# Woody5962/Ranked-List-Truncation

Measured on AMD Instinct MI355X. Metric: ranked-lists/sec (fwd+bwd) at len=300; F1@k vs CPU ref, higher is better.
Workload: dtype f32 (operands, accumulation, storage); products by exact 3xbf16 split, 6 MFMA products, per-product error < 2^-23; 1 GPU; AttnCut + DivLoss(js,f1,augmented) [BASELINE configs[1]], batch 4096 lists/GPU x len 300, full train step incl. Adam and cut metrics; global_batch=4096, seq_len=300, parallelism=dp1

## Files before the change

include/rlt_hip.h:

```cpp
#ifndef RLT_HIP_H
#define RLT_HIP_H

#include <stddef.h>
#include <stdint.h>

#ifdef __cplusplus
extern "C" {
#endif

#define RLT_E_ARG      (-1)
#define RLT_E_SHAPE    (-2)
#define RLT_E_WORKSPACE (-3)
#define RLT_E_ALIGN    (-4)

#define RLT_ABI_VERSION 5
int rlt_abi_version(void);
#define RLT_PRECISION_DEFAULT (-1)
#define RLT_PRECISION_FP32   0
#define RLT_PRECISION_BF16X3 1
#define RLT_PRECISION_BF16X6 2
int rlt_set_precision(int mode);
int rlt_get_precision(void);
const char* rlt_error_string(int code);

// ... 41 lines not shown
                        int32_t* k_out, float* r_k, float* r_best, int32_t* best_k, double* sums,
                        const void* dcg_table, void* ws, size_t ws_bytes, void* stream);

size_t rlt_reward_eval_workspace(int B, int S, int T);
int rlt_reward_eval(const float* labels, const rlt_reward_spec* spec, const float* r_in, int B, int S,
                    const int32_t* k_in, int T, int allow_empty, const void* dcg_table, int accumulate,
                    float* r_at, int32_t* better, float* best, int32_t* best_k,
                    double* curve, double* best_hist, double* sums,
                    void* ws, size_t ws_bytes, void* stream);

size_t rlt_mt_terms_workspace(int B, int S);
int rlt_mt_terms(const float* rerank, const float* cls, const float* labels, int B, int S, float margin,
                 float* terms, void* ws, size_t ws_bytes, void* stream);
int rlt_mt_terms_bwd(const float* cls, const float* labels, const float* terms, int B, int S,
                     float w_rerank, float w_class, const float* gscale,
                     float* d_rerank, float* d_class, void* stream);
int rlt_weighted_sum(const float* const* x, const float* w, int n, float* out, void* stream);

int rlt_cut_metrics(const float* p, const float* labels, const int32_t* k_in, int B, int S,
                    int32_t* k_out, double* f1_out, double* dcg_out, double* sums, void* stream);
int rlt_cut_metrics_ex(const float* p, const float* labels, const int32_t* k_in, int B, int S, double penalty,
                       int32_t* k_out, double* f1_out, double* dcg_out, double* sums, void* stream);

int rlt_task_metrics(const float* labels, const float* pred, int B, int S,
                     double* dcg_out, double* auc_out, double* sums, void* stream);

size_t rlt_truncation_curves_workspace(int B, int S);
int rlt_truncation_curves(const float* labels, int B, int S, double penalty, const void* dcg_table, int accumulate,
                          double* curves, double* best_f1, int32_t* best_f1_k, double* best_dcg, int32_t* best_dcg_k,
                          double* sums, void* ws, size_t ws_bytes, void* stream);

#define RLT_CUT_ARGMAX 0
#define RLT_CUT_PAIR   1
size_t rlt_cut_report_workspace(int B, int S);
int rlt_cut_report(const float* p, int rule, const float* labels, const float* dcg_coef, int B, int S, int metric, float penalty,
                   double metric_penalty, double tau, double sharpen, const void* dcg_table, int accumulate,
                   int32_t* k, float* p_k, float* margin, double* f1, double* dcg, double* best_f1, int32_t* best_f1_k,
                   double* best_dcg, int32_t* best_dcg_k, int32_t* better, double* hist, double* pred_curve, double* reward_curve,
                   double* sums, void* ws, size_t ws_bytes, void* stream);

#define RLT_SWEEP_QUANTILE    0
#define RLT_SWEEP_FIRST_BELOW 1
#define RLT_SWEEP_FIRST_ABOVE 2
#define RLT_SWEEP_COLS        8
size_t rlt_cut_sweep_workspace(int B, int S, int T);
int rlt_cut_sweep(const float* v, int v_stride, int rule, const double* thresholds, int T,
                  const float* labels, int B, int S, double metric_penalty, double beta,
                  const void* dcg_table, int accumulate,
                  int32_t* k , double* curve ,
                  void* ws, size_t ws_bytes, void* stream);

#define RLT_GEMM_RELU       1
#define RLT_GEMM_ACCUMULATE 2
size_t rlt_gemm_workspace(int ta, int tb, int M, int N, int K);
int rlt_gemm(int ta, int tb, int M, int N, int K,
             const float* A, int lda, const float* B, int ldb, float* C, int ldc,
             const float* bias, const float* bias2, int flags,
             void* ws, size_t ws_bytes, int precision, void* stream);
int rlt_gemm_ex(int ta, int tb, int M, int N, int K,
                const float* A, int lda, const float* B, int ldb, float* C, int ldc,
                const float* bias, const float* bias2, int flags,
                const float* relu_mask, int ldmask, float mask_scale, float* colsum_a,
                float drop_p, uint32_t seed,
                void* ws, size_t ws_bytes, int precision, void* stream);

#define RLT_GEMM_NONE   0
#define RLT_GEMM_F32    1
#define RLT_GEMM_3      2
#define RLT_GEMM_3B     3
#define RLT_GEMM_6      4
#define RLT_GEMM_6B     5
#define RLT_GEMM_6C     6
#define RLT_GEMM_6E     7
#define RLT_GEMM_6S     8
typedef struct rlt_gemm_dispatch {
    int family, ta, tb, fast, persistent, ns, kchunk, slab_xcd, epilogue, narrow;
} rlt_gemm_dispatch;
int rlt_gemm_last_dispatch(rlt_gemm_dispatch* out);
#define RLT_GEMM_PTR_A         1
#define RLT_GEMM_PTR_B         2
#define RLT_GEMM_PTR_C         4
#define RLT_GEMM_PTR_BIAS      8
#define RLT_GEMM_PTR_BIAS2     16
#define RLT_GEMM_PTR_BITS_OUT  32
#define RLT_GEMM_PTR_BITS_IN   64
#define RLT_GEMM_PTR_RELU_MASK 128
#define RLT_GEMM_PTR_COLSUM    256
typedef struct rlt_gemm_call {
    int ta, tb, M, N, K, lda, ldb, ldc, flags;
    int aligned16, present, drop, ws_null;
    size_t ws_bytes;
} rlt_gemm_call;
int rlt_gemm_plan(const rlt_gemm_call* call, int precision, rlt_gemm_dispatch* out);

size_t rlt_gemm_bits_words(int M, int N);
int rlt_gemm_bits(int ta, int tb, int M, int N, int K,
                  const float* A, int lda, const float* B, int ldb, float* C, int ldc,
                  const float* bias, int flags, float drop_p, uint32_t seed,
                  uint32_t* relu_bits_out, const uint32_t* mask_bits_in, float mask_scale,
                  int precision, void* stream);
size_t rlt_colsum_workspace(int T, int N);
int rlt_colsum(const float* X, int ldx, int T, int N, float* out, int accumulate,
               void* ws, size_t ws_bytes, void* stream);
int rlt_segment_colsum(const float* X, int ldx, int G, int R, int N, float* out, int ldo,
                       int accumulate, void* stream);

// ... 283 lines not shown
```

ranked-list-truncation_amd/csrc/gemm.hip:

```cpp
#include "common.h"
#include "gemm6s.h"
#include "gemm_plan.h"
#include "split6.h"
#include <type_traits>

namespace {

constexpr int BM = 128, BN = 128, LDT = 132;

struct GemmArgs {
    const float* A; const float* B; float* C;
    const float* bias; const float* bias2;
    int M, N, K, lda, ldb, ldc;
    int vecA, vecB;
    int flags;
    int kchunk;
    float* slab;
    int tiles_m, tiles_n;
    const float* mask; int ldmask;
    float* colsum;
    float* cs_slab;
    float drop_p; uint32_t drop_thr, seed;
    float mask_scale;
    int slab_xcd;
// ... 1238 lines not shown
    __syncthreads();

    int u = 0;
    int nslot = 0; (void)nslot;
    while (true) {
        for (int ti = 0; ti < nt; ++ti) {
            const int b0 = u, b1 = u == 2 ? 0 : u + 1, b2 = b1 == 2 ? 0 : b1 + 1;
            RLT_G6C_STAMP(nslot, 0);
            slot(BoolTag<false>{}, b0, 0, 0, false, 0);
            RLT_G6C_STAMP(nslot, 1);
            __syncthreads();
            RLT_G6C_STAMP(nslot, 2);
            ++nslot;
            RLT_G6C_STAMP(nslot, 0);
            slot(BoolTag<true>{}, b1, b2, b0, ti + 1 < nt || has_next, ti + 2);
            RLT_G6C_STAMP(nslot, 1);
            __syncthreads();
            RLT_G6C_STAMP(nslot, 2);
            ++nslot;
            u = b2;
        }
#ifdef RLT_G6C_NOSTORE
        if (acc[0][0][0] == 123.456f)
#endif
        write_output_t<4>(g, acc, m0 + wm * 64, n0 + wn * 128, true, l31, hh, zslab);
        if (!PERSIST || !has_next) break;
        m0 = nm0; n0 = nn0;
        decode_next();
#pragma unroll
        for (int i = 0; i < 2; ++i)
#pragma unroll
            for (int j = 0; j < 4; ++j)
#pragma unroll
                for (int r = 0; r < 16; ++r) acc[i][j][r] = 0.f;
    }
    if (want_cs) {
        float4* red = reinterpret_cast<float4*>(gsm);
        __syncthreads();
        red[tid] = csum;
        __syncthreads();
        if (tid < 64) {
            float4 t = red[4 * tid];
#pragma unroll
            for (int j = 1; j < 8; ++j) {
                const float4 o = red[(j >> 2) * 256 + 4 * tid + (j & 3)];
                t.x += o.x; t.y += o.y; t.z += o.z; t.w += o.w;
            }
            float* dst = (g.cs_slab ? g.cs_slab + (size_t)zslab * g.M : g.colsum) + m0 + 4 * tid;
            dst[0] = t.x; dst[1] = t.y; dst[2] = t.z; dst[3] = t.w;
        }
    }
}

template <bool KC>
__device__ __forceinline__ size_t off6e(int tid, int ld) {
    if (KC) return (size_t)phys6(tid >> 2) * ld + 4 * (tid & 3);
    return (size_t)(4 * (tid & 3)) * ld + 4 * (tid >> 2);
}
template <bool KC>
__device__ __forceinline__ void load6e(const float* __restrict__ P, int ld, int i, float4& v) {
    v = *reinterpret_cast<const float4*>(P + (size_t)(KC ? 64 * i : i) * ld);
}
template <bool KC>
__device__ __forceinline__ int dst6e(int tid, int p) {
    const int x = tid & 3;
    const int pr = KC ? (tid >> 2) + 64 * p : ((((tid >> 2) * 4) & ~15) | (p << 2) | ((tid >> 2) & 3));
    return pr * 16 + 8 * ((x >> 1) ^ ((pr >> 3) & 1)) + 4 * (x & 1);
}
template <bool KC>
__device__ __forceinline__ void vals6e(const float4 (&v)[4], int p, float& a, float& b, float& c, float& d) {
    if (KC) { a = v[p].x; b = v[p].y; c = v[p].z; d = v[p].w; }
    else {
        const float* f0 = reinterpret_cast<const float*>(&v[0]);
        const float* f1 = reinterpret_cast<const float*>(&v[1]);
        const float* f2 = reinterpret_cast<const float*>(&v[2]);
        const float* f3 = reinterpret_cast<const float*>(&v[3]);
        a = f0[p]; b = f1[p]; c = f2[p]; d = f3[p];
    }
}

template <int NJ>
__device__ __forceinline__ void write_output_simple(const GemmArgs& g, const f32x16 (&acc)[2][NJ], int rbase, int cbase, int l31, int hh, int z) {
    const bool to_slab = g.slab != nullptr;
    float* out = to_slab ? g.slab + (size_t)z * g.M * g.N : g.C;
    const int ldo = to_slab ? g.N : g.ldc;
    const int rb = __builtin_amdgcn_readfirstlane(rbase), cb = __builtin_amdgcn_readfirstlane(cbase);
    const int loff = 4 * hh * ldo + l31;
    const bool relu = !to_slab && (g.flags & RLT_GEMM_RELU), accum = !to_slab && (g.flags & RLT_GEMM_ACCUMULATE);
#pragma unroll
    for (int j = 0; j < NJ; ++j) {
        const int col = cb + j * 32 + l31;
        float bv = 0.f;
        if (!to_slab) {
            if (g.bias) bv += g.bias[col];
            if (g.bias2) bv += g.bias2[col];
        }
#pragma unroll
        for (int i = 0; i < 2; ++i) {
#pragma unroll
            for (int r = 0; r < 16; ++r) {
                const int dr = (r & 3) + 8 * (r >> 2);
                float* base = out + (size_t)(rb + i * 32 + dr) * ldo + (cb + j * 32);
                float v = acc[i][j][r] + bv;
                if (accum) v += base[loff];
                if (relu) v = fmaxf(v, 0.f);
                base[loff] = v;
            }
        }
    }
}

template <bool TA, bool TB, bool PERSIST>
__global__ __launch_bounds__(256, 1) void gemm6e_kernel(GemmArgs g) {
    extern __shared__ __attribute__((aligned(16))) float gsm[];
    uint16_t* lds = reinterpret_cast<uint16_t*>(gsm);
    const int tid = threadIdx.x, lane = tid & 63, wv = __builtin_amdgcn_readfirstlane(tid >> 6);
    const int l31 = lane & 31, hh = lane >> 5;
    const int wm = wv >> 1, wn = wv & 1;
    int bid, zslab;
    decode_block(g, bid, zslab);
    const int tm = bid / g.tiles_n, tn = bid - tm * g.tiles_n;
    int m0 = tm * BM2, n0 = tn * BN2;
    const int kbeg = zslab * g.kchunk;
    const int kend = min(g.K, kbeg + g.kchunk);
    const int nks = (kend - kbeg) / 16;

    f32x16 acc[2][2][4];
#pragma unroll
    for (int i = 0; i < 4; ++i)
#pragma unroll
        for (int j = 0; j < 4; ++j)
#pragma unroll
            for (int r = 0; r < 16; ++r) acc[i >> 1][i & 1][j][r] = 0.f;

    constexpr bool AKC = !TA, BKC = TB;
    const bool want_cs = TA && g.colsum != nullptr && tn == 0;
    float4 csum = make_float4(0.f, 0.f, 0.f, 0.f);
    const int pl = phys6(l31);
    const int csw = 8 * (hh ^ ((pl >> 3) & 1));
    const int arow = (wm * 128 + pl) * 16 + csw, brow = 3 * HB6 + (wn * 128 + pl) * 16 + csw;
    const size_t offA = off6e<AKC>(tid, g.lda), offB = off6e<BKC>(tid, g.ldb);
    int dA[4], dB[4];
#pragma unroll
    for (int p = 0; p < 4; ++p) { dA[p] = dst6e<AKC>(tid, p); dB[p] = 3 * HB6 + dst6e<BKC>(tid, p); }

    int vid = blockIdx.x, nm0 = m0, nn0 = n0;
    bool has_next = false;
    auto decode_next = [&]() {
        const int nwg = g.tiles_m * g.tiles_n;
        vid += gridDim.x;
        has_next = PERSIST && vid < nwg;
        if (has_next) {
            const int q = nwg >> 3, r = nwg & 7, xcd = vid & 7, jj = vid >> 3;
            const int nb = (xcd < r ? xcd * (q + 1) : r * (q + 1) + (xcd - r) * q) + jj;
            const int ntm = nb / g.tiles_n;
            nm0 = ntm * BM2; nn0 = (nb - ntm * g.tiles_n) * BN2;
        }
    };
    auto srcA = [&](int ks) {
        const bool wrap = PERSIST && has_next && ks >= nks;
        const int k0 = kbeg + 16 * (wrap ? ks - nks : min(ks, nks - 1)), mm = wrap ? nm0 : m0;
        return g.A + (AKC ? (size_t)mm * g.lda + k0 : (size_t)k0 * g.lda + mm) + offA;
    };
    auto srcB = [&](int ks) {
        const bool wrap = PERSIST && has_next && ks >= nks;
        const int k0 = kbeg + 16 * (wrap ? ks - nks : min(ks, nks - 1)), nn = wrap ? nn0 : n0;
        return g.B + (BKC ? (size_t)nn * g.ldb + k0 : (size_t)k0 * g.ldb + nn) + offB;
    };
    float4 ra[2][4], rb[2][4];
    auto add_cs = [&](const float4 (&v)[4]) {
#pragma unroll
        for (int i = 0; i < 4; ++i) { csum.x += v[i].x; csum.y += v[i].y; csum.z += v[i].z; csum.w += v[i].w; }
    };
    auto stash_all = [&](uint16_t* wb, const float4 (&va)[4], const float4 (&vb)[4]) {
#pragma unroll
        for (int p = 0; p < 4; ++p) {
            float a, b, c, d;
            uint2 hi, mid, lo;
            vals6e<AKC>(va, p, a, b, c, d);
            split4x3(a, b, c, d, hi, mid, lo);
            *reinterpret_cast<uint2*>(wb + dA[p]) = hi;
            *reinterpret_cast<uint2*>(wb + dA[p] + HB6) = mid;
            *reinterpret_cast<uint2*>(wb + dA[p] + 2 * HB6) = lo;
            vals6e<BKC>(vb, p, a, b, c, d);
            split4x3(a, b, c, d, hi, mid, lo);
            *reinterpret_cast<uint2*>(wb + dB[p]) = hi;
            *reinterpret_cast<uint2*>(wb + dB[p] + HB6) = mid;
            *reinterpret_cast<uint2*>(wb + dB[p] + 2 * HB6) = lo;
        }
    };
    bf16x8 a[4][3], b[2][3];
    auto frag_a = [&](const uint16_t* base, int i, int q) { a[i][q] = *reinterpret_cast<const bf16x8*>(base + arow + q * HB6 + i * 32 * 16); };
    auto frag_b = [&](const uint16_t* base, int j, int q) { b[j & 1][q] = *reinterpret_cast<const bf16x8*>(base + brow + q * HB6 + j * 32 * 16); };

    {
        const float* pa = srcA(0); const float* pb = srcB(0);
#pragma unroll
        for (int i = 0; i < 4; ++i) { load6e<AKC>(pa, g.lda, i, ra[0][i]); load6e<BKC>(pb, g.ldb, i, rb[0][i]); }
        pa = srcA(1); pb = srcB(1);
#pragma unroll
        for (int i = 0; i < 4; ++i) { load6e<AKC>(pa, g.lda, i, ra[1][i]); load6e<BKC>(pb, g.ldb, i, rb[1][i]); }
        if (want_cs) { add_cs(ra[0]); add_cs(ra[1]); }
        stash_all(lds, ra[0], rb[0]);
        stash_all(lds + KB6, ra[1], rb[1]);
        if (PERSIST) decode_next();
        pa = srcA(2); pb = srcB(2);
#pragma unroll
        for (int i = 0; i < 4; ++i) { load6e<AKC>(pa, g.lda, i, ra[0][i]); load6e<BKC>(pb, g.ldb, i, rb[0][i]); }
        pa = srcA(3); pb = srcB(3);
#pragma unroll
        for (int i = 0; i < 4; ++i) { load6e<AKC>(pa, g.lda, i, ra[1][i]); load6e<BKC>(pb, g.ldb, i, rb[1][i]); }
    }
    __syncthreads();
#pragma unroll
    for (int q = 0; q < 3; ++q) { frag_a(lds, 0, q); frag_a(lds, 1, q); frag_b(lds, 0, q); }

    auto slot = [&](auto par_tag, int buf, int wbuf, int nbuf, const float* pa, const float* pb) {
        constexpr int PAR = decltype(par_tag)::value;
        const uint16_t* base = lds + buf * KB6;
        const uint16_t* nbase = lds + nbuf * KB6;
        uint16_t* wb = lds + wbuf * KB6;
        Split6 su;
#define GAP_END __builtin_amdgcn_sched_barrier(0)
#define MM(i_, j_, k_) acc[(i_) >> 1][(i_) & 1][j_] = __builtin_amdgcn_mfma_f32_32x32x16_bf16( \
            a[i_][(k_) == 0 || (k_) == 3 ? 1 : (k_) == 1 ? 2 : 0], b[(j_) & 1][(k_) == 0 || (k_) == 4 ? 1 : (k_) == 2 ? 2 : 0], acc[(i_) >> 1][(i_) & 1][j_], 0, 0, 0)
#define SP(p_, k_) do { float x0_, x1_, x2_, x3_; \
            if ((p_) < 4) vals6e<AKC>(ra[PAR], (p_) & 3, x0_, x1_, x2_, x3_); else vals6e<BKC>(rb[PAR], (p_) & 3, x0_, x1_, x2_, x3_); \
            split6_part(su, x0_, x1_, x2_, x3_, k_); } while (0)
#define ST(p_) do { const int d_ = (p_) < 4 ? dA[(p_) & 3] : dB[(p_) & 3]; \
            *reinterpret_cast<uint2*>(wb + d_) = su.hi; *reinterpret_cast<uint2*>(wb + d_ + HB6) = su.mid; \
            *reinterpret_cast<uint2*>(wb + d_ + 2 * HB6) = su.lo; \
            if ((p_) < 4) { if (AKC) load6e<AKC>(pa, g.lda, (p_) & 3, ra[PAR][(p_) & 3]); \
                            else if ((p_) == 3) { for (int i_ = 0; i_ < 4; ++i_) load6e<AKC>(pa, g.lda, i_, ra[PAR][i_]); } } \
            else { if (BKC) load6e<BKC>(pb, g.ldb, (p_) & 3, rb[PAR][(p_) & 3]); \
                   else if ((p_) == 7) { for (int i_ = 0; i_ < 4; ++i_) load6e<BKC>(pb, g.ldb, i_, rb[PAR][i_]); } } } while (0)
#define RA(i_, q_, n_) frag_a((n_) ? nbase : base, i_, q_)
#define RB(j_, q_, n_) frag_b((n_) ? nbase : base, j_, q_)
#include "gemm6e_slot.inc"
#undef GAP_END
#undef MM
#undef SP
#undef ST
#undef RA
#undef RB
    };

    int u = 0;
    while (true) {
        for (int s = 0; s < nks; s += 2) {
            const int u1 = u == 2 ? 0 : u + 1, u2 = u1 == 2 ? 0 : u1 + 1;
            if (want_cs && s + 2 < nks) add_cs(ra[0]);
            slot(std::integral_constant<int, 0>{}, u, u2, u1, srcA(s + 4), srcB(s + 4));
            __syncthreads();
            if (want_cs && s + 3 < nks) add_cs(ra[1]);
            slot(std::integral_constant<int, 1>{}, u1, u, u2, srcA(s + 5), srcB(s + 5));
            __syncthreads();
            u = u2;
        }
        write_output_simple<4>(g, acc[0], m0 + wm * 128, n0 + wn * 128, l31, hh, zslab);
        write_output_simple<4>(g, acc[1], m0 + wm * 128 + 64, n0 + wn * 128, l31, hh, zslab);
        if (!PERSIST || !has_next) break;
        m0 = nm0; n0 = nn0;
        decode_next();
#pragma unroll
        for (int i = 0; i < 4; ++i)
#pragma unroll
            for (int j = 0; j < 4; ++j)
#pragma unroll
                for (int r = 0; r < 16; ++r) acc[i >> 1][i & 1][j][r] = 0.f;
    }
    if (want_cs) {
        float4* red = reinterpret_cast<float4*>(gsm);
        __syncthreads();
        red[tid] = csum;
        __syncthreads();
        if (tid < 64) {
            float4 t = red[4 * tid];
#pragma unroll
            for (int j = 1; j < 4; ++j) {
                const float4 o = red[4 * tid + j];
                t.x += o.x; t.y += o.y; t.z += o.z; t.w += o.w;
            }
            float* dst = (g.cs_slab ? g.cs_slab + (size_t)zslab * g.M : g.colsum) + m0 + 4 * tid;
            dst[0] = t.x; dst[1] = t.y; dst[2] = t.z; dst[3] = t.w;
        }
    }
}

__device__ __forceinline__ float4 f4add(float4 a, float4 b) { return make_float4(a.x + b.x, a.y + b.y, a.z + b.z, a.w + b.w); }
__global__ __launch_bounds__(256) void splitk_reduce_kernel(GemmArgs g, int nsplit) {
    const size_t mn = (size_t)g.M * g.N;
    const size_t stride = (size_t)gridDim.x * 256;
    if ((g.N & 3) == 0) {
        const float4* slab4 = reinterpret_cast<const float4*>(g.slab);
        const size_t mn4 = mn / 4;
        for (size_t i = (size_t)blockIdx.x * 256 + threadIdx.x; i < mn4; i += stride) {
            float4 a0 = make_float4(0.f, 0.f, 0.f, 0.f), a1 = a0, a2 = a0, a3 = a0;
            int z = 0;
            for (; z + 3 < nsplit; z += 4) {
                a0 = f4add(a0, slab4[(size_t)z * mn4 + i]);
                a1 = f4add(a1, slab4[(size_t)(z + 1) * mn4 + i]);
                a2 = f4add(a2, slab4[(size_t)(z + 2) * mn4 + i]);
                a3 = f4add(a3, slab4[(size_t)(z + 3) * mn4 + i]);
            }
            for (; z < nsplit; ++z) a0 = f4add(a0, slab4[(size_t)z * mn4 + i]);
            const float4 v4 = f4add(f4add(a0, a1), f4add(a2, a3));
            const float v[4] = {v4.x, v4.y, v4.z, v4.w};
            const int row = (int)((4 * i) / g.N), col0 = (int)(4 * i - (size_t)row * g.N);
#pragma unroll
            for (int e = 0; e < 4; ++e) {
                const int col = col0 + e;
                float bv = 0.f;
                if (g.bias) bv += g.bias[col];
                if (g.bias2) bv += g.bias2[col];
                float* dst = g.C + (size_t)row * g.ldc + col;
                *dst = gemm_epilogue(g, v[e], bv, row, col, dst);
            }
        }
    } else {
        for (size_t i = (size_t)blockIdx.x * 256 + threadIdx.x; i < mn; i += stride) {
// ... 161 lines not shown
static int gemm_run(int ta, int tb, int M, int N, int K,
                    const float* A, int lda, const float* B, int ldb, float* C, int ldc,
                    const float* bias, const float* bias2, int flags,
                    const float* relu_mask, int ldmask, float mask_scale, float* colsum_a,
                    float drop_p, uint32_t seed, uint32_t* bits_out, const uint32_t* bits_in,
                    void* ws, size_t ws_bytes, void* stream) {
    rlt_gemm_dispatch_rec = rlt_gemm_dispatch{};
    RLT_CHECK_ARG(A && B && C && M > 0 && N > 0 && K > 0);
    RLT_CHECK_ARG(lda >= (ta ? M : K) && ldb >= (tb ? K : N) && ldc >= N);
    RLT_CHECK_ARG(!relu_mask || ldmask >= N);
    RLT_CHECK_ARG(!colsum_a || ta);
    RLT_CHECK_ARG(drop_p >= 0.f && drop_p < 1.f);

    GemmCall c{};
    c.ta = ta; c.tb = tb; c.M = M; c.N = N; c.K = K; c.lda = lda; c.ldb = ldb; c.ldc = ldc; c.flags = flags;
    auto bit = [](bool on, int b) { return on ? b : 0; };
    c.aligned16 = bit(rlt_aligned16(A), RLT_GEMM_PTR_A) | bit(rlt_aligned16(B), RLT_GEMM_PTR_B) | bit(rlt_aligned16(C), RLT_GEMM_PTR_C) |
                  bit(rlt_aligned16(bias), RLT_GEMM_PTR_BIAS) | bit(rlt_aligned16(bias2), RLT_GEMM_PTR_BIAS2) |
                  bit(rlt_aligned16(bits_out), RLT_GEMM_PTR_BITS_OUT) | bit(rlt_aligned16(bits_in), RLT_GEMM_PTR_BITS_IN);
    c.present = bit(bias, RLT_GEMM_PTR_BIAS) | bit(bias2, RLT_GEMM_PTR_BIAS2) | bit(bits_out, RLT_GEMM_PTR_BITS_OUT) |
                bit(bits_in, RLT_GEMM_PTR_BITS_IN) | bit(relu_mask, RLT_GEMM_PTR_RELU_MASK) | bit(colsum_a, RLT_GEMM_PTR_COLSUM);
    c.drop = drop_p > 0.f; c.ws_null = ws == nullptr; c.ws_bytes = ws_bytes;

    const GemmPlan p = gemm_plan(c);
    if (p.rc) return p.rc;

    hipStream_t st = rlt_stream(stream);
    if (p.d.family == RLT_GEMM_6S) {
        const Gemm6sArgs s6{A, B, C, bias, bias2, M, N, K, lda, ldb, ldc, bits_out, bits_in, mask_scale};
        const int rc = rlt_gemm6s_launch(s6, p, &rlt_gemm_dispatch_rec, st);
        return rc ? rc : RLT_LAUNCH_RESULT();
    }
    const int ns = p.d.ns;
    GemmArgs g;
    g.mask = relu_mask; g.ldmask = ldmask; g.colsum = colsum_a;
    g.bits_out = bits_out; g.bits_in = bits_in; g.ldbits = N;
    g.mask_scale = mask_scale; g.drop_p = drop_p; g.drop_thr = rlt_drop_threshold(drop_p); g.seed = seed;
    g.A = A; g.B = B; g.C = C; g.bias = bias; g.bias2 = bias2;
    g.M = M; g.N = N; g.K = K; g.lda = lda; g.ldb = ldb; g.ldc = ldc;
    g.vecA = (lda % 4 == 0) && rlt_aligned16(A);
    g.vecB = (ldb % 4 == 0) && rlt_aligned16(B);
    g.flags = flags;
    g.tiles_m = p.tiles_m; g.tiles_n = p.tiles_n;
    g.kchunk = p.d.kchunk;
    g.slab_xcd = p.d.slab_xcd;
    g.slab = ns > 1 ? (float*)ws : nullptr;
    g.cs_slab = (ns > 1 && colsum_a) ? (float*)ws + (size_t)ns * M * N : nullptr;
    const int rc = with_layout(ta, tb, [&](auto TA, auto TB) {
        constexpr bool A_ = decltype(TA)::value, B_ = decltype(TB)::value;
        auto go = [&](auto kern) { return launch(kern, p, g, st); };
        const bool persistent = !A_ && p.d.persistent;
        switch (p.d.family) {
        case RLT_GEMM_6E:
            if constexpr (!A_) if (persistent) return go(gemm6e_kernel<A_, B_, true>);
            return go(gemm6e_kernel<A_, B_, false>);
        case RLT_GEMM_6C:
            if constexpr (!A_) if (persistent) return go(gemm6c_kernel<A_, B_, true>);
            return go(gemm6c_kernel<A_, B_, false>);
        case RLT_GEMM_3B:
            if constexpr (!A_) if (persistent) return go(gemm3b_kernel<A_, B_, true>);
            return go(gemm3b_kernel<A_, B_>);
        case RLT_GEMM_6B: return go(gemm6b_kernel<A_, B_>);
        case RLT_GEMM_6: return go(gemm6_kernel<A_, B_>);
        case RLT_GEMM_3: return p.d.fast ? go(gemm3_kernel<A_, B_, true>) : go(gemm3_kernel<A_, B_, false>);
        case RLT_GEMM_F32: return p.d.fast ? go(gemm_kernel<A_, B_, 16, 4, true>) : go(gemm_kernel<A_, B_, 16, 4, false>);
        }
        return (int)RLT_E_ARG;
    });
    if (rc) return rc;
    if (p.reduce)
        hipLaunchKernelGGL(splitk_reduce_kernel, dim3(ew_grid((size_t)M * N)), dim3(256), 0, st, g, ns);
    return RLT_LAUNCH_RESULT();
}

int rlt_gemm_ex(int ta, int tb, int M, int N, int K,
                const float* A, int lda, const float* B, int ldb, float* C, int ldc,
                const float* bias, const float* bias2, int flags,
                const float* relu_mask, int ldmask, float mask_scale, float* colsum_a,
                float drop_p, uint32_t seed,
                void* ws, size_t ws_bytes, int precision, void* stream) {
    RLT_PREC_SCOPE(precision);
    return gemm_run(ta, tb, M, N, K, A, lda, B, ldb, C, ldc, bias, bias2, flags, relu_mask, ldmask, mask_scale, colsum_a,
                    drop_p, seed, nullptr, nullptr, ws, ws_bytes, stream);
}

size_t rlt_gemm_bits_words(int M, int N) { return M > 0 && N > 0 ? (size_t)rlt_cdiv(M, 32) * N : 0; }

int rlt_gemm_bits(int ta, int tb, int M, int N, int K,
                  const float* A, int lda, const float* B, int ldb, float* C, int ldc,
                  const float* bias, int flags, float drop_p, uint32_t seed,
                  uint32_t* relu_bits_out, const uint32_t* mask_bits_in, float mask_scale,
                  int precision, void* stream) {
    RLT_PREC_SCOPE(precision);
    RLT_CHECK_ARG((relu_bits_out != nullptr) != (mask_bits_in != nullptr));
    RLT_CHECK_ARG(!relu_bits_out || (flags & RLT_GEMM_RELU));
    RLT_CHECK_ARG(drop_p == 0.f || relu_bits_out);
    RLT_CHECK_SHAPE(N % 32 == 0);
    return gemm_run(ta, tb, M, N, K, A, lda, B, ldb, C, ldc, bias, nullptr, flags, nullptr, 0, mask_scale, nullptr,
                    drop_p, seed, relu_bits_out, mask_bits_in, nullptr, 0, stream);
}

size_t rlt_colsum_workspace(int T, int N) {
    if (T <= 0 || N <= 0) return 0;
    return (size_t)rlt_cdiv(T, CS_ROWS_PER_WG) * N * sizeof(float);
}

// ... 57 lines not shown
```

ranked-list-truncation_amd/csrc/gemm_plan.hip:

```cpp
#define RLT_HOST_ONLY
#include "gemm_plan.h"
#include "common.h"
#include <stdlib.h>
#include <string.h>

namespace {

struct GemmEnv {
    int mode;
    bool nofast;
    bool no_big;
    int persist;
    bool persist_nn;
    int persist6;
    bool small6;
    bool gemm6c;
    bool gemm6e;
    bool gemm6e_all;
    bool gemm6s;
    int split_kmin;
    int split_target;
    bool no_slab_xcd;
};
const GemmEnv& gemm_env() {
    static const GemmEnv env = [] {
        auto num = [](const char* name, int dflt) { const char* e = getenv(name); return e ? atoi(e) : dflt; };
        GemmEnv v;
        const char* m = getenv("RLT_GEMM_MODE");
        v.mode = !m ? -1 : (!strcmp(m, "bf16x6") || !strcmp(m, "2")) ? 2 : (!strcmp(m, "bf16x3") || !strcmp(m, "1")) ? 1 : 0;
        v.nofast = num("RLT_GEMM_NOFAST", 0) != 0;
        v.no_big = num("RLT_GEMM_NO_BIG", 0) != 0;
        v.persist = num("RLT_GEMM_PERSIST", 256);
        v.persist_nn = num("RLT_GEMM_PERSIST_NN", 0) != 0;
        v.persist6 = num("RLT_GEMM6_PERSIST", 256);
        v.small6 = getenv("RLT_GEMM6_SMALL") != nullptr;
        v.gemm6c = num("RLT_GEMM6C", 1) != 0;
        v.gemm6e = num("RLT_GEMM6E", 1) != 0;
        v.gemm6e_all = num("RLT_GEMM6E_ALL", 0) != 0;
        v.gemm6s = num("RLT_GEMM6S", 1) != 0;
        v.split_kmin = num("RLT_GEMM_SPLIT_KMIN", 1024);
        v.split_target = num("RLT_GEMM_SPLIT_TARGET", 1024);
        v.no_slab_xcd = getenv("RLT_GEMM_NO_SLAB_XCD") != nullptr;
        return v;
    }();
    return env;
}

int wanted_slabs(int M, int N, int K) {
    const GemmEnv& e = gemm_env();
    const long long tiles = (long long)rlt_cdiv(M, 128) * rlt_cdiv(N, 128);
    if (tiles >= 256 || K < e.split_kmin) return 1;
    long long want = e.split_target / tiles > 0 ? e.split_target / tiles : 1;
    const long long per = K >= 4096 ? 512 : 256;
    const long long maxs = K / per > 0 ? K / per : 1;
    if (want > maxs) want = maxs;
    if (want > 256) want = 256;
    if (want >= 8) want = want / 8 * 8;
    return (int)want;
}
size_t slab_bytes(int slabs, int M, int N) { return slabs > 1 ? ((size_t)slabs * M * N + (size_t)slabs * M) * sizeof(float) : 0; }

}

GemmPlan gemm_plan(const GemmCall& c) {
    const GemmEnv& e = gemm_env();
    const int mode = e.mode >= 0 ? e.mode : rlt_precision();
    const int M = c.M, N = c.N, K = c.K;
    const bool ta = c.ta != 0, tb = c.tb != 0;
    auto has = [&](int bit) { return (c.present & bit) != 0; };
    auto al = [&](int bit) { return (c.aligned16 & bit) != 0; };
    const bool bias = has(RLT_GEMM_PTR_BIAS), bias2 = has(RLT_GEMM_PTR_BIAS2), mask = has(RLT_GEMM_PTR_RELU_MASK),
               colsum = has(RLT_GEMM_PTR_COLSUM), bits_out = has(RLT_GEMM_PTR_BITS_OUT), bits_in = has(RLT_GEMM_PTR_BITS_IN);
    const bool relu = (c.flags & RLT_GEMM_RELU) != 0, accumulate = (c.flags & RLT_GEMM_ACCUMULATE) != 0, drop = c.drop != 0;
    const bool vec = c.lda % 4 == 0 && al(RLT_GEMM_PTR_A) && c.ldb % 4 == 0 && al(RLT_GEMM_PTR_B);

    GemmPlan p{};
    const int want = bits_out || bits_in ? 1 : wanted_slabs(M, N, K);
    p.ws_bytes = slab_bytes(want, M, N);
    int ns = want;
    if (ns > 1 && (c.ws_null || c.ws_bytes < p.ws_bytes)) {
        if (c.ws_null && c.ws_bytes == 0) ns = 1;
        else { p.rc = RLT_E_WORKSPACE; return p; }
    }
    const int kchunk = rlt_cdiv(rlt_cdiv(K, ns), 32) * 32;
    ns = rlt_cdiv(K, kchunk);
    const int slab_xcd = ns > 1 && ns % 8 == 0 && !e.no_slab_xcd;

    const bool wide = N % 256 == 0;
    const bool gemm6s = mode == 2 && e.gemm6s && !ta && ns == 1 && !mask && !colsum && !drop && !accumulate &&
        (!bits_in || (!bias && !bias2 && !relu)) && !(bits_out && bits_in) &&
        (K == 256 || K == 128) && (wide || (K == 128 && N % 128 == 0 && !bits_out && !bits_in)) && N <= 256 * 256 && M >= 32 * 256 &&
        vec && c.ldc % 4 == 0 && al(RLT_GEMM_PTR_C) && (!bias || al(RLT_GEMM_PTR_BIAS)) && (!bias2 || al(RLT_GEMM_PTR_BIAS2)) &&
        (!bits_out || al(RLT_GEMM_PTR_BITS_OUT)) && (!bits_in || al(RLT_GEMM_PTR_BITS_IN)) &&
        (size_t)c.lda * 4 * 32 < (1u << 31) && (size_t)c.ldc * 4 * 32 < (1u << 31);
    const bool tile6 = mode == 2 && vec && M % 256 == 0 && N % 128 == 0 && K % 32 == 0;
    const bool big6 = tile6 && wide && !e.small6;
    const bool pipe6 = big6 && e.gemm6c && kchunk >= 64 && (K % kchunk == 0 || K % kchunk >= 64);
    const bool plain_epilogue = !mask && !bits_in && !bits_out && !drop;
    const bool big3 = mode == 1 && !e.no_big && vec && M % 256 == 0 && N % 256 == 0 && K % 32 == 0;
    const int family = gemm6s ? RLT_GEMM_6S
                     : pipe6 ? (e.gemm6e && plain_epilogue && (ta || K >= 1024 || e.gemm6e_all) ? RLT_GEMM_6E : RLT_GEMM_6C)
                     : big6 ? RLT_GEMM_6B
                     : tile6 ? RLT_GEMM_6
                     : big3 ? RLT_GEMM_3B
                     : mode == 1 ? RLT_GEMM_3 : RLT_GEMM_F32;
    const GemmFamily& f = GEMM_FAMILY[family];
    p.wg = f.wg;
    p.lds_bytes = f.lds;
    p.reduce = ns > 1;

    if (family == RLT_GEMM_6S) {
        if (bits_out && !relu) { p.rc = -1; return p; }
        const int narrow = !wide;
        const int npanel = N / (narrow ? 128 : 256), nblk = (M + 31) / 32;
        int nstream = 256 / npanel;
        if (nstream < 1) nstream = 1;
        if (nstream > nblk) nstream = nblk;
        p.tiles_m = nstream; p.tiles_n = npanel;
        p.grid_x = npanel * nstream; p.grid_z = 1;
        p.lds_bytes = K == 256 ? GEMM6S_LDS_K256 : GEMM6S_LDS_K128;
        p.d = rlt_gemm_dispatch{family, 0, tb, 1, 0, 1, K, 0, bits_in ? 3 : bits_out ? 2 : relu ? 1 : 0, narrow};
        return p;
    }
    p.tiles_m = rlt_cdiv(M, f.bm); p.tiles_n = rlt_cdiv(N, f.bn);
    const long long tiles = (long long)p.tiles_m * p.tiles_n;
    const bool small = family == RLT_GEMM_F32 || family == RLT_GEMM_3;
    const bool fast = !small || (!e.nofast && vec && K % 4 == 0 && K >= 4 && (!ta || (M % 4 == 0 && M >= 4)) && (tb || (N % 4 == 0 && N >= 4)));
    const int wgs = family == RLT_GEMM_3B ? e.persist : e.persist6;
    const bool persistent = !ta && ns == 1 && wgs > 0 && wgs % 8 == 0 && tiles > wgs &&
        (family == RLT_GEMM_3B ? (tb || (e.persist_nn && !bits_in)) && K / 32 >= 2 : family == RLT_GEMM_6C || family == RLT_GEMM_6E);
    p.grid_x = persistent ? wgs : (unsigned)(tiles * (slab_xcd ? ns : 1));
    p.grid_z = slab_xcd ? 1 : ns;
    p.d = rlt_gemm_dispatch{family, ta, tb, fast, persistent, ns, kchunk, slab_xcd, 0, 0};
    return p;
}

extern "C" {

size_t rlt_gemm_workspace(int ta, int tb, int M, int N, int K) {
    (void)ta; (void)tb;
    if (M <= 0 || N <= 0 || K <= 0) return 0;
    return slab_bytes(wanted_slabs(M, N, K), M, N);
}

int rlt_gemm_plan(const rlt_gemm_call* c, int precision, rlt_gemm_dispatch* out) {
    RLT_PREC_SCOPE(precision);
    RLT_CHECK_ARG(c && out && c->M > 0 && c->N > 0 && c->K > 0);
    RLT_CHECK_ARG(c->lda >= (c->ta ? c->M : c->K) && c->ldb >= (c->tb ? c->K : c->N) && c->ldc >= c->N);
    RLT_CHECK_ARG(!(c->present & RLT_GEMM_PTR_COLSUM) || c->ta);
    const GemmPlan p = gemm_plan(*c);
    *out = p.d;
    return p.rc;
}

}
```

ranked-list-truncation_amd/csrc/path.hip:

```cpp
#include "common.h"
#include <stdio.h>
#include <stdlib.h>

namespace {

constexpr size_t ALIGN = 256;
inline size_t rup(size_t b) { return (b + ALIGN - 1) / ALIGN * ALIGN; }

struct Cursor {
    uint8_t* base; size_t off, cap;
    explicit Cursor(void* p, size_t cap_ = (size_t)-1) : base((uint8_t*)p), off(0), cap(cap_) {}
    template <typename T = float> T* take(size_t bytes) {
        T* p = (T*)(base ? base + off : nullptr);
#ifdef RLT_BOUNDS_CHECK
        if (base && cap != (size_t)-1 && off + bytes > cap) {
            fprintf(stderr, "rlt bounds check: region of %zu bytes at offset %zu leaves a %zu-byte buffer\n", bytes, off, cap);
            abort();
        }
#endif
        off += rup(bytes);
        return p;
    }
};

// ... 137 lines not shown
}
inline int pack2(const float* a, const float* b, size_t n, float* out, hipStream_t st) {
    const int grid = (int)((2 * n + 255) / 256 < 512 ? (2 * n + 255) / 256 : 512);
    hipLaunchKernelGGL(pack2_kernel, dim3(grid), dim3(256), 0, st, a, b, n, out);
    return RLT_LAUNCH_RESULT();
}
inline int unpack2(const float* in, size_t n, float* a, float* b, hipStream_t st) {
    const int grid = (int)((2 * n + 255) / 256 < 512 ? (2 * n + 255) / 256 : 512);
    hipLaunchKernelGGL(unpack2_kernel, dim3(grid), dim3(256), 0, st, in, n, a, b);
    return RLT_LAUNCH_RESULT();
}

int lstm_layer_fwd(const float* x, int I, const rlt_lstm_layer_weights& w, int S, int B, float* gates, float* c, float* h,
                   const LstmScratch& sc, void* stream, const rlt_sparse_batch* sp = nullptr) {
    const int T = S * B;
    if (sp) {
        RLT_TRY(rlt_sparse_inproj_fwd(sp, S, B, w.w_ih[0], w.w_ih[1], w.b_ih[0], w.b_hh[0], w.b_ih[1], w.b_hh[1], gates, stream));
        return rlt_bilstm_rec_fwd(gates, w.w_hh[0], w.w_hh[1], S, B, h, c, RLT_PRECISION_DEFAULT, stream);
    }
    if (I <= 3)
        return rlt_bilstm_rec_fwd_x(x, I, w.w_ih[0], w.b_ih[0], w.b_hh[0], w.w_ih[1], w.b_ih[1], w.b_hh[1], w.w_hh[0], w.w_hh[1],
                                    S, B, gates, h, c, RLT_PRECISION_DEFAULT, stream);
    hipStream_t st = rlt_stream(stream);
    RLT_TRY(pack2(w.w_ih[0], w.w_ih[1], (size_t)512 * I, sc.wcat, st));
    RLT_TRY(pack2(w.b_ih[0], w.b_ih[1], 512, sc.bcat, st));
    RLT_TRY(pack2(w.b_hh[0], w.b_hh[1], 512, sc.bcat + 1024, st));
    RLT_TRY(rlt_gemm_ex(0, 1, T, 1024, I, x, I, sc.wcat, I, gates, 1024, sc.bcat, sc.bcat + 1024, 0, nullptr, 0, 1.f, nullptr,
                        0.f, 0u, sc.ws, sc.ws_bytes, RLT_PRECISION_DEFAULT, stream));
    return rlt_bilstm_rec_fwd(gates, w.w_hh[0], w.w_hh[1], S, B, h, c, RLT_PRECISION_DEFAULT, stream);
}

int lstm_layer_bwd(const float* x, int I, const rlt_lstm_layer_weights& w, const float* h, float* gates, const float* c,
                   const float* dh, int S, int B, float* dx, const rlt_lstm_layer_grads& g, const LstmScratch& sc, void* stream,
                   const rlt_sparse_batch* sp = nullptr, void* sp_ws = nullptr, size_t sp_ws_bytes = 0) {
    const int T = S * B;
    hipStream_t st = rlt_stream(stream);
    RLT_TRY(rlt_bilstm_rec_bwd(gates, c, w.w_hh[0], w.w_hh[1], dh, S, B, RLT_PRECISION_DEFAULT, stream));
    const float* dA = gates;
    if (sp) {
        RLT_TRY(rlt_sparse_inproj_bwd(sp, S, B, dA, g.w_ih[0], g.w_ih[1], g.b_ih[0], g.b_hh[0], g.b_ih[1], g.b_hh[1],
                                      sp_ws, sp_ws_bytes, stream));
    } else if (I <= 3) {
        RLT_TRY(rlt_narrow_dw(dA, 1024, x, I, I, T, 1024, sc.dwcat, sc.dbcat, sc.ws, sc.ws_bytes, stream));
    } else {
        RLT_TRY(gemm(1, 0, 1024, I, T, dA, 1024, x, I, sc.dwcat, I, nullptr, 0, sc.dbcat, sc.ws, sc.ws_bytes, stream));
    }
    if (!sp) {
        RLT_TRY(unpack2(sc.dwcat, (size_t)512 * I, g.w_ih[0], g.w_ih[1], st));
        RLT_TRY(unpack2(sc.dbcat, 512, g.b_ih[0], g.b_ih[1], st));
        RLT_TRY(unpack2(sc.dbcat, 512, g.b_hh[0], g.b_hh[1], st));
    }
    if (S > 1) {
        const int K = T - B;
        RLT_TRY(gemm(1, 0, 512, 128, K, dA + (size_t)B * 1024, 1024, h, 256, g.w_hh[0], 128, nullptr, 0, nullptr, sc.ws, sc.ws_bytes, stream));
        RLT_TRY(gemm(1, 0, 512, 128, K, dA + 512, 1024, h + (size_t)B * 256 + 128, 256, g.w_hh[1], 128, nullptr, 0, nullptr, sc.ws, sc.ws_bytes, stream));
    } else {
        RLT_TRY((int)hipMemsetAsync(g.w_hh[0], 0, 512 * 128 * sizeof(float), st));
        RLT_TRY((int)hipMemsetAsync(g.w_hh[1], 0, 512 * 128 * sizeof(float), st));
    }
    if (dx) {
        RLT_TRY(pack2(w.w_ih[0], w.w_ih[1], (size_t)512 * I, sc.wcat, st));
        RLT_TRY(gemm(0, 0, T, I, 1024, dA, 1024, sc.wcat, I, dx, I, nullptr, 0, nullptr, sc.ws, sc.ws_bytes, stream));
    }
    return 0;
}

bool lstm_weights_ok(const rlt_lstm_layer_weights& w) {
    for (int d = 0; d < 2; ++d)
        if (!w.w_ih[d] || !w.w_hh[d] || !w.b_ih[d] || !w.b_hh[d]) return false;
    return true;
}
bool lstm_grads_ok(const rlt_lstm_layer_grads& g) {
    for (int d = 0; d < 2; ++d)
        if (!g.w_ih[d] || !g.w_hh[d] || !g.b_ih[d] || !g.b_hh[d]) return false;
    return true;
}

}

extern "C" {

size_t rlt_workspace_bytes(int op, int S, int B, int E, int H, int FF, int train_dropout, int precision) {
    RLT_PREC_SCOPE_SZ(precision);
    if (op == RLT_OP_ENCODER_STASH || op == RLT_OP_ENCODER_BWD_WS || op == RLT_OP_ENCODER_FWD_WS) {
        EncDims d;
        if (enc_dims(S, B, E, H, FF, d)) return 0;
        if (op == RLT_OP_ENCODER_STASH) return enc_stash(d, nullptr).bytes;
        if (op == RLT_OP_ENCODER_FWD_WS) return rup(enc_gemm_ws(d)) + rup(enc_fwd_images_scratch(d, train_dropout ? 0.5f : 0.f));
        return enc_scratch(d, train_dropout != 0, nullptr).bytes;
    }
    if (op == RLT_OP_BILSTM_STASH || op == RLT_OP_BILSTM_WS) {
        if (S <= 0 || B <= 0 || E <= 0) return 0;
        const size_t T = (size_t)S * B;
        return op == RLT_OP_BILSTM_STASH ? lstm_stash(T, nullptr).bytes : lstm_scratch(T, E, nullptr).bytes;
    }
    return 0;
}

int rlt_encoder_layer_fwd(const float* x, const rlt_encoder_weights* w, int S, int B, int E, int H, int FF, float eps,
                          float drop_p, const uint32_t* seeds, float* y, void* stash, size_t stash_bytes,
                          void* ws, size_t ws_bytes, int precision, void* stream) {
    RLT_PREC_SCOPE(precision);
    RLT_CHECK_ARG(x && w && y && stash && drop_p >= 0.f && drop_p < 1.f && (drop_p == 0.f || seeds));
    RLT_CHECK_ARG(w->in_proj_weight && w->in_proj_bias && w->out_proj_weight && w->out_proj_bias && w->norm1_weight &&
                  w->norm1_bias && w->linear1_weight && w->linear1_bias && w->linear2_weight && w->linear2_bias &&
                  w->norm2_weight && w->norm2_bias);
    EncDims d;
    RLT_TRY(enc_dims(S, B, E, H, FF, d));
// ... 132 lines not shown
```

Measured before the change: 24880 lists/s.

## Add N=128 tile variant of gemm6e kernel for LSTM recurrent weight-grad GEMMs

Templates the 6-product bf16-split gemm6e kernel on an N-tile width so it can run 256x128 tiles, and adds a matching MFMA/split schedule include for the narrower tile. The planner routes transposed-A GEMMs flagged RLT_GEMM_TILE_N128 (the two 512x128xK w_hh gradient GEMMs in the BiLSTM backward) to this kernel instead of the older gemm6 path. The aim is to give these narrow-N, long-K reductions the pipelined split-K kernel without wasting half of a 256-wide tile. It adds a second hand-scheduled slot sequence and a new env knob, and it rejects the narrow path for the non-transposed instantiation.

Result: no change. 24950 lists/s, median of 6 (+0.3%).

```diff
diff --git a/include/rlt_hip.h b/include/rlt_hip.h
--- a/include/rlt_hip.h
+++ b/include/rlt_hip.h
@@ -117,6 +117,7 @@
 
 #define RLT_GEMM_RELU       1
 #define RLT_GEMM_ACCUMULATE 2
+#define RLT_GEMM_TILE_N128  4
 size_t rlt_gemm_workspace(int ta, int tb, int M, int N, int K);
 int rlt_gemm(int ta, int tb, int M, int N, int K,
              const float* A, int lda, const float* B, int ldb, float* C, int ldc,
diff --git a/ranked-list-truncation_amd/csrc/gemm.hip b/ranked-list-truncation_amd/csrc/gemm.hip
--- a/ranked-list-truncation_amd/csrc/gemm.hip
+++ b/ranked-list-truncation_amd/csrc/gemm.hip
@@ -1314,19 +1314,21 @@
     }
 }
 
-template <bool KC>
+template <bool KC, int NB = 4>
 __device__ __forceinline__ size_t off6e(int tid, int ld) {
     if (KC) return (size_t)phys6(tid >> 2) * ld + 4 * (tid & 3);
-    return (size_t)(4 * (tid & 3)) * ld + 4 * (tid >> 2);
-}
-template <bool KC>
+    return (size_t)(4 * (tid & 3)) * ld + (NB == 4 ? 4 : 2) * (tid >> 2);
+}
+template <bool KC, int NB = 4>
 __device__ __forceinline__ void load6e(const float* __restrict__ P, int ld, int i, float4& v) {
-    v = *reinterpret_cast<const float4*>(P + (size_t)(KC ? 64 * i : i) * ld);
-}
-template <bool KC>
+    if (NB == 4) v = *reinterpret_cast<const float4*>(P + (size_t)(KC ? 64 * i : i) * ld);
+    else if (KC) { if (i < NB) v = *reinterpret_cast<const float4*>(P + (size_t)(64 * i) * ld); }
+    else { const float2 t = *reinterpret_cast<const float2*>(P + (size_t)i * ld); v.x = t.x; v.y = t.y; }
+}
+template <bool KC, int NB = 4>
 __device__ __forceinline__ int dst6e(int tid, int p) {
     const int x = tid & 3;
-    const int pr = KC ? (tid >> 2) + 64 * p : ((((tid >> 2) * 4) & ~15) | (p << 2) | ((tid >> 2) & 3));
+    const int pr = KC ? (tid >> 2) + 64 * p : NB == 4 ? ((((tid >> 2) * 4) & ~15) | (p << 2) | ((tid >> 2) & 3)) : phys6(2 * (tid >> 2) + (p & 1));
     return pr * 16 + 8 * ((x >> 1) ^ ((pr >> 3) & 1)) + 4 * (x & 1);
 }
 template <bool KC>
@@ -1372,7 +1374,7 @@
     }
 }
 
-template <bool TA, bool TB, bool PERSIST>
+template <bool TA, bool TB, bool PERSIST, int NB = 4>
 __global__ __launch_bounds__(256, 1) void gemm6e_kernel(GemmArgs g) {
     extern __shared__ __attribute__((aligned(16))) float gsm[];
     uint16_t* lds = reinterpret_cast<uint16_t*>(gsm);
@@ -1382,16 +1384,17 @@
     int bid, zslab;
     decode_block(g, bid, zslab);
     const int tm = bid / g.tiles_n, tn = bid - tm * g.tiles_n;
-    int m0 = tm * BM2, n0 = tn * BN2;
+    constexpr int BNT = 64 * NB;
+    int m0 = tm * BM2, n0 = tn * BNT;
     const int kbeg = zslab * g.kchunk;
     const int kend = min(g.K, kbeg + g.kchunk);
     const int nks = (kend - kbeg) / 16;
 
-    f32x16 acc[2][2][4];
+    f32x16 acc[2][2][NB];
 #pragma unroll
     for (int i = 0; i < 4; ++i)
 #pragma unroll
-        for (int j = 0; j < 4; ++j)
+        for (int j = 0; j < NB; ++j)
 #pragma unroll
             for (int r = 0; r < 16; ++r) acc[i >> 1][i & 1][j][r] = 0.f;
 
@@ -1400,11 +1403,11 @@
     float4 csum = make_float4(0.f, 0.f, 0.f, 0.f);
     const int pl = phys6(l31);
     const int csw = 8 * (hh ^ ((pl >> 3) & 1));
-    const int arow = (wm * 128 + pl) * 16 + csw, brow = 3 * HB6 + (wn * 128 + pl) * 16 + csw;
-    const size_t offA = off6e<AKC>(tid, g.lda), offB = off6e<BKC>(tid, g.ldb);
+    const int arow = (wm * 128 + pl) * 16 + csw, brow = 3 * HB6 + (wn * 32 * NB + pl) * 16 + csw;
+    const size_t offA = off6e<AKC>(tid, g.lda), offB = off6e<BKC, NB>(tid, g.ldb);
     int dA[4], dB[4];
 #pragma unroll
-    for (int p = 0; p < 4; ++p) { dA[p] = dst6e<AKC>(tid, p); dB[p] = 3 * HB6 + dst6e<BKC>(tid, p); }
+    for (int p = 0; p < 4; ++p) { dA[p] = dst6e<AKC>(tid, p); dB[p] = 3 * HB6 + dst6e<BKC, NB>(tid, p); }
 
     int vid = blockIdx.x, nm0 = m0, nn0 = n0;
     bool has_next = false;
@@ -1416,7 +1419,7 @@
             const int q = nwg >> 3, r = nwg & 7, xcd = vid & 7, jj = vid >> 3;
             const int nb = (xcd < r ? xcd * (q + 1) : r * (q + 1) + (xcd - r) * q) + jj;
             const int ntm = nb / g.tiles_n;
-            nm0 = ntm * BM2; nn0 = (nb - ntm * g.tiles_n) * BN2;
+            nm0 = ntm * BM2; nn0 = (nb - ntm * g.tiles_n) * BNT;
         }
     };
     auto srcA = [&](int ks) {
@@ -1444,6 +1447,7 @@
             *reinterpret_cast<uint2*>(wb + dA[p]) = hi;
             *reinterpret_cast<uint2*>(wb + dA[p] + HB6) = mid;
             *reinterpret_cast<uint2*>(wb + dA[p] + 2 * HB6) = lo;
+            if (p >= NB) continue;
             vals6e<BKC>(vb, p, a, b, c, d);
             split4x3(a, b, c, d, hi, mid, lo);
             *reinterpret_cast<uint2*>(wb + dB[p]) = hi;
@@ -1458,20 +1462,20 @@
     {
         const float* pa = srcA(0); const float* pb = srcB(0);
 #pragma unroll
-        for (int i = 0; i < 4; ++i) { load6e<AKC>(pa, g.lda, i, ra[0][i]); load6e<BKC>(pb, g.ldb, i, rb[0][i]); }
+        for (int i = 0; i < 4; ++i) { load6e<AKC>(pa, g.lda, i, ra[0][i]); load6e<BKC, NB>(pb, g.ldb, i, rb[0][i]); }
         pa = srcA(1); pb = srcB(1);
 #pragma unroll
-        for (int i = 0; i < 4; ++i) { load6e<AKC>(pa, g.lda, i, ra[1][i]); load6e<BKC>(pb, g.ldb, i, rb[1][i]); }
+        for (int i = 0; i < 4; ++i) { load6e<AKC>(pa, g.lda, i, ra[1][i]); load6e<BKC, NB>(pb, g.ldb, i, rb[1][i]); }
         if (want_cs) { add_cs(ra[0]); add_cs(ra[1]); }
         stash_all(lds, ra[0], rb[0]);
         stash_all(lds + KB6, ra[1], rb[1]);
         if (PERSIST) decode_next();
         pa = srcA(2); pb = srcB(2);
 #pragma unroll
-        for (int i = 0; i < 4; ++i) { load6e<AKC>(pa, g.lda, i, ra[0][i]); load6e<BKC>(pb, g.ldb, i, rb[0][i]); }
+        for (int i = 0; i < 4; ++i) { load6e<AKC>(pa, g.lda, i, ra[0][i]); load6e<BKC, NB>(pb, g.ldb, i, rb[0][i]); }
         pa = srcA(3); pb = srcB(3);
 #pragma unroll
-        for (int i = 0; i < 4; ++i) { load6e<AKC>(pa, g.lda, i, ra[1][i]); load6e<BKC>(pb, g.ldb, i, rb[1][i]); }
+        for (int i = 0; i < 4; ++i) { load6e<AKC>(pa, g.lda, i, ra[1][i]); load6e<BKC, NB>(pb, g.ldb, i, rb[1][i]); }
     }
     __syncthreads();
 #pragma unroll
@@ -1494,11 +1498,15 @@
             *reinterpret_cast<uint2*>(wb + d_ + 2 * HB6) = su.lo; \
             if ((p_) < 4) { if (AKC) load6e<AKC>(pa, g.lda, (p_) & 3, ra[PAR][(p_) & 3]); \
                             else if ((p_) == 3) { for (int i_ = 0; i_ < 4; ++i_) load6e<AKC>(pa, g.lda, i_, ra[PAR][i_]); } } \
-            else { if (BKC) load6e<BKC>(pb, g.ldb, (p_) & 3, rb[PAR][(p_) & 3]); \
-                   else if ((p_) == 7) { for (int i_ = 0; i_ < 4; ++i_) load6e<BKC>(pb, g.ldb, i_, rb[PAR][i_]); } } } while (0)
+            else { if (BKC) load6e<BKC, NB>(pb, g.ldb, (p_) & 3, rb[PAR][(p_) & 3]); \
+                   else if ((p_) == 3 + NB) { for (int i_ = 0; i_ < 4; ++i_) load6e<BKC, NB>(pb, g.ldb, i_, rb[PAR][i_]); } } } while (0)
 #define RA(i_, q_, n_) frag_a((n_) ? nbase : base, i_, q_)
 #define RB(j_, q_, n_) frag_b((n_) ? nbase : base, j_, q_)
+    if constexpr (NB == 4) {
 #include "gemm6e_slot.inc"
+    } else {
+#include "gemm6e_n128_slot.inc"
+    }
 #undef GAP_END
 #undef MM
 #undef SP
@@ -1519,15 +1527,15 @@
             __syncthreads();
             u = u2;
         }
-        write_output_simple<4>(g, acc[0], m0 + wm * 128, n0 + wn * 128, l31, hh, zslab);
-        write_output_simple<4>(g, acc[1], m0 + wm * 128 + 64, n0 + wn * 128, l31, hh, zslab);
+        write_output_simple<NB>(g, acc[0], m0 + wm * 128, n0 + wn * 32 * NB, l31, hh, zslab);
+        write_output_simple<NB>(g, acc[1], m0 + wm * 128 + 64, n0 + wn * 32 * NB, l31, hh, zslab);
         if (!PERSIST || !has_next) break;
         m0 = nm0; n0 = nn0;
         decode_next();
 #pragma unroll
         for (int i = 0; i < 4; ++i)
 #pragma unroll
-            for (int j = 0; j < 4; ++j)
+            for (int j = 0; j < NB; ++j)
 #pragma unroll
                 for (int r = 0; r < 16; ++r) acc[i >> 1][i & 1][j][r] = 0.f;
     }
@@ -1795,6 +1803,8 @@
         const bool persistent = !A_ && p.d.persistent;
         switch (p.d.family) {
         case RLT_GEMM_6E:
+            if constexpr (A_) if (p.d.narrow) return go(gemm6e_kernel<A_, B_, false, 2>);
+            if (p.d.narrow) return (int)RLT_E_ARG;
             if constexpr (!A_) if (persistent) return go(gemm6e_kernel<A_, B_, true>);
             return go(gemm6e_kernel<A_, B_, false>);
         case RLT_GEMM_6C:
diff --git a/ranked-list-truncation_amd/csrc/gemm6e_n128_slot.inc b/ranked-list-truncation_amd/csrc/gemm6e_n128_slot.inc
--- /dev/null
+++ b/ranked-list-truncation_amd/csrc/gemm6e_n128_slot.inc
@@ -0,0 +1,48 @@
+MM(0, 0, 0); GAP_END; SP(0, 0); RA(3, 1, 0); GAP_END;
+MM(0, 0, 1); GAP_END; SP(0, 1); RA(3, 2, 0); GAP_END;
+MM(0, 0, 2); GAP_END; SP(0, 2); RB(1, 2, 0); GAP_END;
+MM(0, 0, 3); GAP_END; SP(0, 3); GAP_END;
+MM(0, 0, 4); GAP_END; SP(0, 4); GAP_END;
+MM(0, 0, 5); GAP_END; SP(0, 5); RA(2, 0, 0); GAP_END;
+MM(1, 0, 0); GAP_END; ST(0); GAP_END;
+MM(1, 0, 1); GAP_END; RA(2, 1, 0); RA(2, 2, 0); GAP_END;
+MM(1, 0, 2); GAP_END; SP(1, 0); GAP_END;
+MM(1, 0, 3); GAP_END; SP(1, 1); GAP_END;
+MM(1, 0, 4); GAP_END; SP(1, 2); GAP_END;
+MM(1, 0, 5); GAP_END; SP(1, 3); GAP_END;
+MM(2, 0, 0); GAP_END; SP(1, 4); GAP_END;
+MM(2, 0, 1); GAP_END; SP(1, 5); RA(3, 0, 0); GAP_END;
+MM(2, 0, 2); GAP_END; ST(1); GAP_END;
+MM(2, 0, 3); GAP_END; RB(1, 0, 0); RB(1, 1, 0); GAP_END;
+MM(2, 0, 4); GAP_END; SP(2, 0); GAP_END;
+MM(2, 0, 5); GAP_END; SP(2, 1); GAP_END;
+MM(3, 0, 0); GAP_END; SP(2, 2); GAP_END;
+MM(3, 0, 1); GAP_END; SP(2, 3); GAP_END;
+MM(3, 0, 2); GAP_END; SP(2, 4); GAP_END;
+MM(3, 0, 3); GAP_END; SP(2, 5); GAP_END;
+MM(3, 0, 4); GAP_END; ST(2); GAP_END;
+MM(3, 0, 5); GAP_END; GAP_END;
+MM(0, 1, 0); GAP_END; SP(3, 0); GAP_END;
+MM(0, 1, 1); GAP_END; SP(3, 1); GAP_END;
+MM(0, 1, 2); GAP_END; SP(3, 2); GAP_END;
+MM(0, 1, 3); GAP_END; SP(3, 3); GAP_END;
+MM(0, 1, 4); GAP_END; SP(3, 4); GAP_END;
+MM(0, 1, 5); GAP_END; SP(3, 5); RB(0, 0, 1); GAP_END;
+MM(1, 1, 0); GAP_END; ST(3); GAP_END;
+MM(1, 1, 1); GAP_END; RB(0, 1, 1); RB(0, 2, 1); GAP_END;
+MM(1, 1, 2); GAP_END; SP(4, 0); GAP_END;
+MM(1, 1, 3); GAP_END; SP(4, 1); GAP_END;
+MM(1, 1, 4); GAP_END; SP(4, 2); GAP_END;
+MM(1, 1, 5); GAP_END; SP(4, 3); GAP_END;
+MM(2, 1, 0); GAP_END; SP(4, 4); GAP_END;
+MM(2, 1, 1); GAP_END; SP(4, 5); RA(0, 0, 1); GAP_END;
+MM(2, 1, 2); GAP_END; ST(4); GAP_END;
+MM(2, 1, 3); GAP_END; RA(0, 1, 1); RA(0, 2, 1); GAP_END;
+MM(2, 1, 4); GAP_END; SP(5, 0); GAP_END;
+MM(2, 1, 5); GAP_END; SP(5, 1); GAP_END;
+MM(3, 1, 0); GAP_END; SP(5, 2); GAP_END;
+MM(3, 1, 1); GAP_END; SP(5, 3); GAP_END;
+MM(3, 1, 2); GAP_END; SP(5, 4); GAP_END;
+MM(3, 1, 3); GAP_END; SP(5, 5); RA(1, 0, 1); GAP_END;
+MM(3, 1, 4); GAP_END; ST(5); GAP_END;
+MM(3, 1, 5); GAP_END; RA(1, 1, 1); RA(1, 2, 1); GAP_END;
diff --git a/ranked-list-truncation_amd/csrc/gemm_plan.hip b/ranked-list-truncation_amd/csrc/gemm_plan.hip
--- a/ranked-list-truncation_amd/csrc/gemm_plan.hip
+++ b/ranked-list-truncation_amd/csrc/gemm_plan.hip
@@ -17,6 +17,7 @@
     bool gemm6c;
     bool gemm6e;
     bool gemm6e_all;
+    bool gemm6e_n128;
     bool gemm6s;
     int split_kmin;
     int split_target;
@@ -37,6 +38,7 @@
         v.gemm6c = num("RLT_GEMM6C", 1) != 0;
         v.gemm6e = num("RLT_GEMM6E", 1) != 0;
         v.gemm6e_all = num("RLT_GEMM6E_ALL", 0) != 0;
+        v.gemm6e_n128 = num("RLT_GEMM6E_N128", 1) != 0;
         v.gemm6s = num("RLT_GEMM6S", 1) != 0;
         v.split_kmin = num("RLT_GEMM_SPLIT_KMIN", 1024);
         v.split_target = num("RLT_GEMM_SPLIT_TARGET", 1024);
@@ -97,10 +99,13 @@
     const bool big6 = tile6 && wide && !e.small6;
     const bool pipe6 = big6 && e.gemm6c && kchunk >= 64 && (K % kchunk == 0 || K % kchunk >= 64);
     const bool plain_epilogue = !mask && !bits_in && !bits_out && !drop;
+    const bool narrow6e = tile6 && !wide && ta && (c.flags & RLT_GEMM_TILE_N128) && !e.small6 && e.gemm6c && e.gemm6e && e.gemm6e_n128 &&
+        plain_epilogue && kchunk >= 64 && (K % kchunk == 0 || K % kchunk >= 64);
     const bool big3 = mode == 1 && !e.no_big && vec && M % 256 == 0 && N % 256 == 0 && K % 32 == 0;
     const int family = gemm6s ? RLT_GEMM_6S
                      : pipe6 ? (e.gemm6e && plain_epilogue && (ta || K >= 1024 || e.gemm6e_all) ? RLT_GEMM_6E : RLT_GEMM_6C)
                      : big6 ? RLT_GEMM_6B
+                     : narrow6e ? RLT_GEMM_6E
                      : tile6 ? RLT_GEMM_6
                      : big3 ? RLT_GEMM_3B
                      : mode == 1 ? RLT_GEMM_3 : RLT_GEMM_F32;
@@ -122,7 +127,7 @@
         p.d = rlt_gemm_dispatch{family, 0, tb, 1, 0, 1, K, 0, bits_in ? 3 : bits_out ? 2 : relu ? 1 : 0, narrow};
         return p;
     }
-    p.tiles_m = rlt_cdiv(M, f.bm); p.tiles_n = rlt_cdiv(N, f.bn);
+    p.tiles_m = rlt_cdiv(M, f.bm); p.tiles_n = rlt_cdiv(N, narrow6e ? 128 : f.bn);
     const long long tiles = (long long)p.tiles_m * p.tiles_n;
     const bool small = family == RLT_GEMM_F32 || family == RLT_GEMM_3;
     const bool fast = !small || (!e.nofast && vec && K % 4 == 0 && K >= 4 && (!ta || (M % 4 == 0 && M >= 4)) && (tb || (N % 4 == 0 && N >= 4)));
@@ -131,7 +136,7 @@
         (family == RLT_GEMM_3B ? (tb || (e.persist_nn && !bits_in)) && K / 32 >= 2 : family == RLT_GEMM_6C || family == RLT_GEMM_6E);
     p.grid_x = persistent ? wgs : (unsigned)(tiles * (slab_xcd ? ns : 1));
     p.grid_z = slab_xcd ? 1 : ns;
-    p.d = rlt_gemm_dispatch{family, ta, tb, fast, persistent, ns, kchunk, slab_xcd, 0, 0};
+    p.d = rlt_gemm_dispatch{family, ta, tb, fast, persistent, ns, kchunk, slab_xcd, 0, narrow6e};
     return p;
 }
 
diff --git a/ranked-list-truncation_amd/csrc/path.hip b/ranked-list-truncation_amd/csrc/path.hip
--- a/ranked-list-truncation_amd/csrc/path.hip
+++ b/ranked-list-truncation_amd/csrc/path.hip
@@ -213,8 +213,8 @@
     }
     if (S > 1) {
         const int K = T - B;
-        RLT_TRY(gemm(1, 0, 512, 128, K, dA + (size_t)B * 1024, 1024, h, 256, g.w_hh[0], 128, nullptr, 0, nullptr, sc.ws, sc.ws_bytes, stream));
-        RLT_TRY(gemm(1, 0, 512, 128, K, dA + 512, 1024, h + (size_t)B * 256 + 128, 256, g.w_hh[1], 128, nullptr, 0, nullptr, sc.ws, sc.ws_bytes, stream));
+        RLT_TRY(gemm(1, 0, 512, 128, K, dA + (size_t)B * 1024, 1024, h, 256, g.w_hh[0], 128, nullptr, RLT_GEMM_TILE_N128, nullptr, sc.ws, sc.ws_bytes, stream));
+        RLT_TRY(gemm(1, 0, 512, 128, K, dA + 512, 1024, h + (size_t)B * 256 + 128, 256, g.w_hh[1], 128, nullptr, RLT_GEMM_TILE_N128, nullptr, sc.ws, sc.ws_bytes, stream));
     } else {
         RLT_TRY((int)hipMemsetAsync(g.w_hh[0], 0, 512 * 128 * sizeof(float), st));
         RLT_TRY((int)hipMemsetAsync(g.w_hh[1], 0, 512 * 128 * sizeof(float), st));
```
